# gau-nernst/llama-x

Hardware: AMD Instinct MI355X
Metric: train tokens/sec Llama-3.1-8B seq4096 at 1/2/4/8 MI355X; p50 step ms (higher is better)
Workload: dtype bf16; 1 GPU; Llama-3.1-8B text-only LoRA r=16 bf16, seq=4096, 1 sequence per GPU, causal mask, base+LM head frozen (BASELINE.json configs[1]); random-init weights at 8B dimensions; seq_len=4096, parallelism=dp1, launch=hipGraph replay (fwd+bwd+AdamW), lm_head_rows=labelled only

## Files before the change

llama-x_amd/csrc/common.h:

```cpp
#pragma once
#include <hip/hip_runtime.h>
#include <stdint.h>
#include <stdarg.h>
#include <stdio.h>

#define LLX_OK 0
#define LLX_ERR_ARG -1
#define LLX_ERR_LAUNCH -2
#define LLX_ERR_UNSUPPORTED -3

void llx_set_error(const char* fmt, ...);

#define LLX_REQUIRE(cond, ...)            \
  do {                                    \
    if (!(cond)) {                        \
      llx_set_error(__VA_ARGS__);         \
      return LLX_ERR_ARG;                 \
    }                                     \
  } while (0)

#define LLX_LAUNCH_CHECK(name)                                              \
  do {                                                                      \
    hipError_t e__ = hipGetLastError();                                     \
    if (e__ != hipSuccess) {                                                \
      llx_set_error("%s: launch failed: %s", name, hipGetErrorString(e__)); \
      return LLX_ERR_LAUNCH;                                                \
    }                                                                       \
  } while (0)

typedef uint16_t bf16_t;

typedef __attribute__((ext_vector_type(8))) __bf16 bf16x8_t;
typedef __attribute__((ext_vector_type(4))) float f32x4_t;
typedef __attribute__((ext_vector_type(16))) float f32x16_t;
typedef __attribute__((ext_vector_type(4))) int i32x4_t;
typedef __attribute__((ext_vector_type(16))) int i32x16_t;
typedef __attribute__((ext_vector_type(4))) short s16x4_t;
typedef __attribute__((ext_vector_type(4))) uint32_t u32x4_t;
typedef __attribute__((ext_vector_type(2))) uint32_t u32x2_t;

#define LLX_WAVE 64

__device__ __forceinline__ float bf2f(bf16_t v) { return __uint_as_float(((uint32_t)v) << 16); }
__device__ __forceinline__ bf16_t f2bf(float f) {
  __bf16 b = (__bf16)f;
  return __builtin_bit_cast(bf16_t, b);
}
__device__ __forceinline__ uint32_t pack_bf2(float lo, float hi) {
  return (uint32_t)f2bf(lo) | ((uint32_t)f2bf(hi) << 16);
}
__device__ __forceinline__ float bflo(uint32_t w) { return __uint_as_float(w << 16); }
__device__ __forceinline__ float bfhi(uint32_t w) { return __uint_as_float(w & 0xffff0000u); }

__device__ __forceinline__ float wave_sum(float v) {
#pragma unroll
  for (int o = 32; o > 0; o >>= 1) v += __shfl_xor(v, o, 64);
  return v;
}
__device__ __forceinline__ float wave_max(float v) {
#pragma unroll
  for (int o = 32; o > 0; o >>= 1) v = fmaxf(v, __shfl_xor(v, o, 64));
  return v;
}

__device__ __forceinline__ float block_sum(float v, float* red) {
  v = wave_sum(v);
  const int lane = threadIdx.x & 63, w = threadIdx.x >> 6, nw = (blockDim.x + 63) >> 6;
  __syncthreads();
  if (lane == 0) red[w] = v;
  __syncthreads();
  float t = 0.f;
  for (int i = 0; i < nw; ++i) t += red[i];
  return t;
}
__device__ __forceinline__ float block_max(float v, float* red) {
  v = wave_max(v);
  const int lane = threadIdx.x & 63, w = threadIdx.x >> 6, nw = (blockDim.x + 63) >> 6;
  __syncthreads();
  if (lane == 0) red[w] = v;
  __syncthreads();
  float t = red[0];
  for (int i = 1; i < nw; ++i) t = fmaxf(t, red[i]);
  return t;
}

static inline int64_t cdiv64(int64_t a, int64_t b) { return (a + b - 1) / b; }

__device__ __forceinline__ float sigmoidf_(float x) { return __builtin_amdgcn_rcpf(1.f + __expf(-x)); }
__device__ __forceinline__ u32x4_t swiglu_fwd8(const u32x4_t& gv, const u32x4_t& uv) {
  u32x4_t o;
#pragma unroll
  for (int e = 0; e < 4; ++e) {
    const float g0 = bflo(gv[e]), g1 = bfhi(gv[e]);
    const float s0 = bf2f(f2bf(g0 * sigmoidf_(g0))), s1 = bf2f(f2bf(g1 * sigmoidf_(g1)));
    o[e] = pack_bf2(s0 * bflo(uv[e]), s1 * bfhi(uv[e]));
  }
  return o;
}
__device__ __forceinline__ void swiglu_bwd8(const u32x4_t& dv, const u32x4_t& gv, const u32x4_t& uv, u32x4_t& og, u32x4_t& ou) {
#pragma unroll
  for (int e = 0; e < 4; ++e) {
    float dgs[2], dus[2];
#pragma unroll
    for (int p = 0; p < 2; ++p) {
      const float gg = p ? bfhi(gv[e]) : bflo(gv[e]);
      const float uu = p ? bfhi(uv[e]) : bflo(uv[e]);
      const float dd = p ? bfhi(dv[e]) : bflo(dv[e]);
      const float sg = sigmoidf_(gg);
      const float silu = bf2f(f2bf(gg * sg));
      dus[p] = dd * silu;
      const float ds = bf2f(f2bf(dd * uu));
      dgs[p] = ds * (sg * (1.f + gg * (1.f - sg)));
    }
    og[e] = pack_bf2(dgs[0], dgs[1]);
    ou[e] = pack_bf2(dus[0], dus[1]);
  }
}

__device__ __forceinline__ u32x4_t rope8(const u32x4_t& v, const f32x4_t& t0, const f32x4_t& t1, float sign) {
  const float cs[4] = {t0[0], t0[2], t1[0], t1[2]};
  const float sn[4] = {t0[1] * sign, t0[3] * sign, t1[1] * sign, t1[3] * sign};
  u32x4_t o;
#pragma unroll
  for (int e = 0; e < 4; ++e) {
    const float x0 = bflo(v[e]), x1 = bfhi(v[e]);
    o[e] = pack_bf2(x0 * cs[e] - x1 * sn[e], x1 * cs[e] + x0 * sn[e]);
  }
  return o;
}

__device__ __forceinline__ u32x4_t rope8(const u32x4_t& v, const float* __restrict__ tp, float sign) {
  const f32x4_t t0 = *reinterpret_cast<const f32x4_t*>(tp);
  const f32x4_t t1 = *reinterpret_cast<const f32x4_t*>(tp + 4);
  const float cs[4] = {t0[0], t0[2], t1[0], t1[2]};
  const float sn[4] = {t0[1] * sign, t0[3] * sign, t1[1] * sign, t1[3] * sign};
  u32x4_t o;
#pragma unroll
  for (int e = 0; e < 4; ++e) {
    const float x0 = bflo(v[e]), x1 = bfhi(v[e]);
    o[e] = pack_bf2(x0 * cs[e] - x1 * sn[e], x1 * cs[e] + x0 * sn[e]);
  }
  return o;
}

typedef __attribute__((ext_vector_type(8))) short llx_s16x8_t;
template <int OFF>
__device__ __forceinline__ void lds_tr_read(s16x4_t& dst, uint32_t addr) {
  asm volatile("ds_read_b64_tr_b16 %0, %1 offset:%2" : "=v"(dst) : "v"(addr), "n"(OFF));
}
__device__ __forceinline__ void lds_tr_read_rt(s16x4_t& dst, uint32_t addr, int off) {
  asm volatile("ds_read_b64_tr_b16 %0, %1 offset:%2" : "=v"(dst) : "v"(addr), "n"(off));
}
template <int N>
__device__ __forceinline__ void lds_tr_wait4(s16x4_t& a, s16x4_t& b, s16x4_t& c, s16x4_t& d) {
  asm volatile("s_waitcnt lgkmcnt(%4)" : "+v"(a), "+v"(b), "+v"(c), "+v"(d) : "n"(N));
  __builtin_amdgcn_sched_barrier(0);
}
template <int N>
__device__ __forceinline__ void lds_tr_wait8(s16x4_t (&c)[4], s16x4_t (&d)[4]) {
  asm volatile("s_waitcnt lgkmcnt(%8)" : "+v"(c[0]), "+v"(c[1]), "+v"(c[2]), "+v"(c[3]), "+v"(d[0]), "+v"(d[1]), "+v"(d[2]), "+v"(d[3]) : "n"(N));
  __builtin_amdgcn_sched_barrier(0);
}
__device__ __forceinline__ bf16x8_t frag_of(const s16x4_t& lo, const s16x4_t& hi) {
  const llx_s16x8_t v = {lo[0], lo[1], lo[2], lo[3], hi[0], hi[1], hi[2], hi[3]};
  return __builtin_bit_cast(bf16x8_t, v);
}

typedef __attribute__((address_space(3))) void llx_lds_void;
__device__ __forceinline__ __amdgpu_buffer_rsrc_t lds_dma_rsrc(const void* base, uint32_t bytes) {
  return __builtin_amdgcn_make_buffer_rsrc(const_cast<void*>(base), 0, (int)bytes, 0x00020000);
}
__device__ __forceinline__ void lds_dma16(__amdgpu_buffer_rsrc_t rsrc, llx_lds_void* dst, uint32_t lane_off, uint32_t wave_off) {
  __builtin_amdgcn_raw_ptr_buffer_load_lds(rsrc, dst, 16, (int)lane_off, (int)wave_off, 0, 0);
}
```

llama-x_amd/csrc/gemm_bf16.hip:

```cpp
#include "common.h"
#include <type_traits>
#include <mutex>

#define BM 256
#define BN 256
#define BK 64
#define STAGE_BYTES (2 * 256 * BK * 2)
#define A_TILE_BYTES (256 * BK * 2)
#define EPI_ROW_BYTES 528
#define GEMM_LDS_BYTES (256 * EPI_ROW_BYTES)

enum { EPI_NONE = 0, EPI_RESIDUAL = 1, EPI_BIAS = 2, EPI_BIAS_GELU = 3, EPI_COLSCALE = 4, EPI_ROWCOLSCALE = 5, EPI_SWIGLU_BWD = 6, EPI_SWIGLU_FWD = 7, EPI_ROPE = 8, EPI_SPLITK = 9, EPI_ROWCOLSCALE_F32 = 10 };

struct GemmArgs {
  const bf16_t* A; const bf16_t* B; bf16_t* C;
  const bf16_t* A2; const bf16_t* B2;
  const bf16_t* E;
  const bf16_t* E2;
  int64_t lda, ldb, ldc, lde, lda2, ldb2;
  int M, N, K, K2;
  int grid_m, grid_n;
  int col0, col_end;
  const bf16_t* sa; const bf16_t* sb;
  const float* rope;
  int rope_S, rope_cols;
  const int* m_valid;
  float* C32;
  int splits;
};

typedef __attribute__((address_space(3))) void lds_void;
typedef const __attribute__((address_space(1))) void gbl_void;

__device__ __forceinline__ float gelu_erf(float x) { return 0.5f * x * (1.0f + erff(x * 0.70710678118654752440f)); }

template <int EPI, bool I8, int PIPE, int BNT = 256>
__global__ __launch_bounds__(512, 2) void gemm_nt_kernel(const GemmArgs g) {
  static_assert(BNT == 256 || BNT == 128, "tile width");
  static_assert(PIPE == 1, "the four-phase main loop is the only one");
  static_assert(BNT == 256 || EPI != EPI_SWIGLU_FWD, "the SwiGLU-forward epilogue needs the full tile");
  constexpr int ESZ = I8 ? 1 : 2;
  constexpr int TK = 128 / ESZ;
  constexpr int WNG = BNT / 64;
  constexpr int WR = 256 / (8 / WNG);
  constexpr int MI = WR / 16;
  constexpr int MH = MI / 2;
  constexpr int BSI = BNT / 64;
  constexpr int EROW = BNT * 2 + 16;
  extern __shared__ __attribute__((aligned(16))) char smem[];
  const int tid = threadIdx.x;
  const int lane = tid & 63;
  const int wave = __builtin_amdgcn_readfirstlane(tid >> 6);
  const int wm = wave / WNG, wn = wave % WNG;

  int grid_m = g.grid_m;
  if (g.m_valid != nullptr) grid_m = min(grid_m, (*g.m_valid + BM - 1) / BM);
  const int nsplit = EPI == EPI_SPLITK ? g.splits : 1;
  const int nwg = grid_m * g.grid_n * nsplit;
  int bid = blockIdx.x;
  if (bid >= nwg) return;
  {
    const int q = nwg >> 3, r = nwg & 7, x = bid & 7;
    bid = (x < r ? x * (q + 1) : r * (q + 1) + (x - r) * q) + (bid >> 3);
  }
  const int split = EPI == EPI_SPLITK ? bid / (grid_m * g.grid_n) : 0;
  if constexpr (EPI == EPI_SPLITK) bid -= split * (grid_m * g.grid_n);
  const int GROUP_M = 4;
  const int width = GROUP_M * g.grid_n;
  const int group = bid / width;
  const int gsz = min(grid_m - group * GROUP_M, GROUP_M);
  const int pid_m = group * GROUP_M + ((bid % width) % gsz);
  const int pid_n = (bid % width) / gsz;
  constexpr bool SPLITN = EPI == EPI_SWIGLU_FWD;
  const int halfN = g.N >> 1;
  const int m0 = pid_m * BM, n0 = SPLITN ? pid_n * (BN / 2) : g.col0 + pid_n * BNT;
  auto col_of = [&](int nl) { return SPLITN ? (nl < BN / 2 ? n0 + nl : halfN + n0 + nl - BN / 2) : min(n0 + nl, g.col_end - 1); };

  const int srow = tid >> 3;
  const int schunk = (tid & 7) ^ ((tid >> 4) & 7);
  int arow[4], brow[4];
#pragma unroll
  for (int i = 0; i < 4; ++i) {
    arow[i] = min(m0 + i * 64 + srow, g.M - 1);
    brow[i] = SPLITN ? (i < 2 ? n0 + i * 64 + srow : halfN + n0 + (i - 2) * 64 + srow) : min(n0 + (i % BSI) * 64 + srow, g.col_end - 1);
  }
  const int nk1 = g.K / TK / nsplit;
  const int nk = nk1 + g.K2 / 64;
  const int kofs = split * nk1;

  uint32_t aoff[4], boff[4];
#pragma unroll
  for (int i = 0; i < 4; ++i) {
    aoff[i] = (uint32_t)((int64_t)arow[i] * g.lda * ESZ + schunk * 16);
    boff[i] = (uint32_t)((int64_t)brow[i] * g.ldb * ESZ + schunk * 16);
  }
  const __amdgpu_buffer_rsrc_t rsA = lds_dma_rsrc(g.A, (uint32_t)(((int64_t)(g.M - 1) * g.lda + g.K) * ESZ));
  const __amdgpu_buffer_rsrc_t rsB = lds_dma_rsrc(g.B, (uint32_t)(((int64_t)(g.N - 1) * g.ldb + g.K) * ESZ));

  const int frow = lane & 15;
  const int fsw = (lane >> 1) & 7;
  const int fq = lane >> 4;
  const int a_base = (wm * WR + frow) * 128;
  const int b_base = (wn * 64 + frow) * 128;
  const int slot0 = ((0 * 4 + fq) ^ fsw) * 16;
  const int slot1 = ((1 * 4 + fq) ^ fsw) * 16;

  using acc_t = typename std::conditional<I8, i32x4_t, f32x4_t>::type;
  acc_t acc[MI][4];
#pragma unroll
  for (int i = 0; i < MI; ++i)
#pragma unroll
    for (int j = 0; j < 4; ++j) acc[i][j] = acc_t{0, 0, 0, 0};

  auto stage_q = [&](auto steady_tag, int kt, int which) {
    constexpr bool steady = decltype(steady_tag)::value;
    if constexpr (!steady) {
      if (kt >= nk) return;
    }
    const int half = which >> 1, hi = which & 1;
    const int np = half ? BSI / 2 : 2;
    char* sT = smem + (kt & 1) * STAGE_BYTES + half * A_TILE_BYTES + hi * np * 8192;
    if (steady || kt < nk1) {
      const uint32_t koff = (uint32_t)(kt + kofs) * 128;
#pragma unroll
      for (int j = 0; j < 2; ++j) {
        if (j < np) {
          if (half) lds_dma16(rsB, (llx_lds_void*)(sT + (j * 512 + wave * 64) * 16), boff[np * hi + j], koff);
          else lds_dma16(rsA, (llx_lds_void*)(sT + (j * 512 + wave * 64) * 16), aoff[2 * hi + j], koff);
        }
      }
    } else {
      const char* base = (const char*)(half ? g.B2 : g.A2) + (int64_t)(kt - nk1) * 128;
      const int64_t l = (half ? g.ldb2 : g.lda2) * 2;
#pragma unroll
      for (int j = 0; j < 2; ++j) {
        if (j < np) {
          const char* src = base + (int64_t)(half ? brow[np * hi + j] : arow[2 * hi + j]) * l + schunk * 16;
          __builtin_amdgcn_global_load_lds((gbl_void*)src, (lds_void*)(sT + (j * 512 + wave * 64) * 16), 16, 0, 0);
        }
      }
    }
  };
  auto mfma_t = [&](auto ext_tag, const i32x4_t& b, const i32x4_t& a, acc_t& c) {
    constexpr bool ext_phase = decltype(ext_tag)::value;
    if constexpr (I8) {
      if constexpr (ext_phase) {
        f32x4_t cf = __builtin_bit_cast(f32x4_t, c);
        cf = __builtin_amdgcn_mfma_f32_16x16x32_bf16(__builtin_bit_cast(bf16x8_t, b), __builtin_bit_cast(bf16x8_t, a), cf, 0, 0, 0);
        c = __builtin_bit_cast(acc_t, cf);
      } else {
        c = __builtin_amdgcn_mfma_i32_16x16x64_i8(b, a, c, 0, 0, 0);
      }
    } else {
      c = __builtin_amdgcn_mfma_f32_16x16x32_bf16(__builtin_bit_cast(bf16x8_t, b), __builtin_bit_cast(bf16x8_t, a), c, 0, 0, 0);
    }
  };
  auto dequant_in_place = [&]() {
    if constexpr (I8) {
      float sbv[4][4], rsv[MI];
#pragma unroll
      for (int ni = 0; ni < 4; ++ni)
#pragma unroll
        for (int e = 0; e < 4; ++e) sbv[ni][e] = bf2f(g.sb[col_of(wn * 64 + ni * 16 + fq * 4 + e)]);
#pragma unroll
      for (int mi = 0; mi < MI; ++mi) rsv[mi] = bf2f(g.sa[min(m0 + wm * WR + mi * 16 + frow, g.M - 1)]);
#pragma unroll
      for (int mi = 0; mi < MI; ++mi) {
        const float rs = rsv[mi];
#pragma unroll
        for (int ni = 0; ni < 4; ++ni) {
          f32x4_t cf;
#pragma unroll
          for (int e = 0; e < 4; ++e) cf[e] = bf2f(f2bf(((float)acc[mi][ni][e] * rs) * sbv[ni][e]));
          acc[mi][ni] = __builtin_bit_cast(acc_t, cf);
        }
      }
    }
  };
  {
    const std::false_type guarded{};
    stage_q(guarded, 0, 0); stage_q(guarded, 0, 1); stage_q(guarded, 0, 2); stage_q(guarded, 0, 3);
    stage_q(guarded, 1, 2); stage_q(guarded, 1, 3); stage_q(guarded, 1, 0);
  }
  auto ktile = [&](int kt, auto ext_tag, auto steady_tag) __attribute__((always_inline)) {
    constexpr bool steady = decltype(steady_tag)::value;
    auto mfma = [&](const i32x4_t& b, const i32x4_t& a, acc_t& c) { mfma_t(ext_tag, b, a, c); };
    const char* sA = smem + (kt & 1) * STAGE_BYTES;
    const char* sB = sA + A_TILE_BYTES;
    if (steady || kt + 1 < nk) {
      if constexpr (BSI == 4) asm volatile("s_waitcnt vmcnt(6)" ::: "memory");
      else asm volatile("s_waitcnt vmcnt(4)" ::: "memory");
    } else asm volatile("s_waitcnt vmcnt(0)" ::: "memory");
    __builtin_amdgcn_s_barrier();
    asm volatile("" ::: "memory");
    stage_q(steady_tag, kt + 1, 1);
    i32x4_t bfr[2][4], af[2 * MH];
#pragma unroll
    for (int ks = 0; ks < 2; ++ks)
#pragma unroll
      for (int ni = 0; ni < 4; ++ni) bfr[ks][ni] = *reinterpret_cast<const i32x4_t*>(sB + b_base + ni * 16 * 128 + (ks ? slot1 : slot0));
#pragma unroll
    for (int ks = 0; ks < 2; ++ks)
#pragma unroll
      for (int m4 = 0; m4 < MH; ++m4) af[ks * MH + m4] = *reinterpret_cast<const i32x4_t*>(sA + a_base + m4 * 16 * 128 + (ks ? slot1 : slot0));
    __builtin_amdgcn_s_setprio(1);
#pragma unroll
    for (int ks = 0; ks < 2; ++ks)
#pragma unroll
      for (int m4 = 0; m4 < MH; ++m4)
#pragma unroll
        for (int n2 = 0; n2 < 2; ++n2) mfma(bfr[ks][n2], af[ks * MH + m4], acc[m4][n2]);
    __builtin_amdgcn_s_setprio(0);
    asm volatile("" ::: "memory");
    __builtin_amdgcn_s_barrier();
    asm volatile("" ::: "memory");
    stage_q(steady_tag, kt + 2, 2);
    __builtin_amdgcn_s_setprio(1);
#pragma unroll
    for (int ks = 0; ks < 2; ++ks)
#pragma unroll
      for (int m4 = 0; m4 < MH; ++m4)
#pragma unroll
        for (int n2 = 0; n2 < 2; ++n2) mfma(bfr[ks][2 + n2], af[ks * MH + m4], acc[m4][2 + n2]);
    __builtin_amdgcn_s_setprio(0);
    stage_q(steady_tag, kt + 2, 3);
#pragma unroll
    for (int ks = 0; ks < 2; ++ks)
#pragma unroll
      for (int m4 = 0; m4 < MH; ++m4) af[ks * MH + m4] = *reinterpret_cast<const i32x4_t*>(sA + a_base + (MH + m4) * 16 * 128 + (ks ? slot1 : slot0));
    __builtin_amdgcn_s_setprio(1);
#pragma unroll
    for (int ks = 0; ks < 2; ++ks)
#pragma unroll
      for (int m4 = 0; m4 < MH; ++m4)
#pragma unroll
        for (int n2 = 0; n2 < 2; ++n2) mfma(bfr[ks][2 + n2], af[ks * MH + m4], acc[MH + m4][2 + n2]);
    __builtin_amdgcn_s_setprio(0);
    asm volatile("" ::: "memory");
    __builtin_amdgcn_s_barrier();
    asm volatile("" ::: "memory");
    stage_q(steady_tag, kt + 2, 0);
    __builtin_amdgcn_s_setprio(1);
#pragma unroll
    for (int ks = 0; ks < 2; ++ks)
#pragma unroll
      for (int m4 = 0; m4 < MH; ++m4)
#pragma unroll
        for (int n2 = 0; n2 < 2; ++n2) mfma(bfr[ks][n2], af[ks * MH + m4], acc[MH + m4][n2]);
    __builtin_amdgcn_s_setprio(0);
  };
  const int nk_main = I8 ? nk1 : nk;
  int kt = 0;
#pragma unroll 1
  for (; kt + 2 < nk1; ++kt) ktile(kt, std::false_type{}, std::true_type{});
#pragma unroll 1
  for (; kt < nk_main; ++kt) ktile(kt, std::false_type{}, std::false_type{});
  if constexpr (I8) {
    if (nk > nk1) {
      dequant_in_place();
      for (kt = nk1; kt < nk; ++kt) ktile(kt, std::true_type{}, std::false_type{});
    }
  }
  __syncthreads();

  if constexpr (EPI == EPI_SPLITK) {
    float* P = g.C32 + (int64_t)split * g.M * g.N;
#pragma unroll
    for (int mi = 0; mi < MI; ++mi) {
      const int gm = m0 + wm * WR + mi * 16 + frow;
#pragma unroll
      for (int ni = 0; ni < 4; ++ni) {
        const int gn = n0 + wn * 64 + ni * 16 + fq * 4;
        if (gm < g.M && gn < g.col_end) *reinterpret_cast<f32x4_t*>(P + (int64_t)gm * g.N + gn) = acc[mi][ni];
      }
    }
    return;
  }
  if constexpr (EPI == EPI_ROWCOLSCALE_F32) {
    static_assert(I8, "int8 kernel only");
    float* Cf = reinterpret_cast<float*>(g.C);
    const float* saf = reinterpret_cast<const float*>(g.sa);
    const float* sbf = reinterpret_cast<const float*>(g.sb);
#pragma unroll
    for (int mi = 0; mi < MI; ++mi) {
      const int gm = m0 + wm * WR + mi * 16 + frow;
      const float rs = saf[min(gm, g.M - 1)];
#pragma unroll
      for (int ni = 0; ni < 4; ++ni) {
        const int gn = n0 + wn * 64 + ni * 16 + fq * 4;
        if (gm < g.M && gn < g.col_end) {
          const f32x4_t cs = *reinterpret_cast<const f32x4_t*>(sbf + gn);
          f32x4_t c;
#pragma unroll
          for (int e = 0; e < 4; ++e) c[e] = ((float)acc[mi][ni][e] * rs) * cs[e];
          *reinterpret_cast<f32x4_t*>(Cf + (int64_t)gm * g.ldc + gn) = c;
        }
      }
    }
    return;
  }
  constexpr int NIT = BNT / 16;
  constexpr int EB0 = (EPI == EPI_SWIGLU_BWD || EPI == EPI_ROPE) ? 4 : 8;
  constexpr int EB = EB0 < NIT / 2 ? EB0 : NIT / 2;
  constexpr bool AUX = EPI == EPI_RESIDUAL || EPI == EPI_BIAS || EPI == EPI_BIAS_GELU || EPI == EPI_SWIGLU_BWD || EPI == EPI_ROPE || EPI == EPI_COLSCALE;
  auto load_aux = [&](int it0, u32x4_t (&aux0)[EB], u32x4_t (&aux1)[EB]) {
    if constexpr (AUX) {
#pragma unroll
      for (int j = 0; j < EB; ++j) {
        const int q = (it0 + j) * 512 + tid;
        const int row = q / (BNT / 8), cc = q % (BNT / 8);
        const int gmc = min(m0 + row, g.M - 1), gnc = min(n0 + cc * 8, g.col_end - 8);
        if constexpr (EPI == EPI_RESIDUAL) {
          aux0[j] = *reinterpret_cast<const u32x4_t*>(g.E + (int64_t)gmc * g.lde + gnc);
        } else if constexpr (EPI == EPI_SWIGLU_BWD) {
          aux0[j] = *reinterpret_cast<const u32x4_t*>(g.E + (int64_t)gmc * g.lde + gnc);
          aux1[j] = *reinterpret_cast<const u32x4_t*>(g.E + (int64_t)gmc * g.lde + g.N + gnc);
        } else if constexpr (EPI == EPI_ROPE) {
          const float* tp = g.rope + ((int64_t)(gmc % g.rope_S) * 64 + ((gnc & 127) >> 1)) * 2;
          aux0[j] = *reinterpret_cast<const u32x4_t*>(tp);
          aux1[j] = *reinterpret_cast<const u32x4_t*>(tp + 4);
        } else {
          aux0[j] = *reinterpret_cast<const u32x4_t*>(g.E + gnc);
        }
      }
    }
  };
  u32x4_t auxA0[EB], auxA1[EB], auxB0[EB], auxB1[EB];
  if constexpr (!SPLITN) load_aux(0, auxA0, auxA1);
  float sbv[4][4], rsv[MI];
  if constexpr (I8) {
    if (g.K2 <= 0) {
#pragma unroll
      for (int ni = 0; ni < 4; ++ni)
#pragma unroll
        for (int e = 0; e < 4; ++e) sbv[ni][e] = bf2f(g.sb[col_of(wn * 64 + ni * 16 + fq * 4 + e)]);
#pragma unroll
      for (int mi = 0; mi < MI; ++mi) rsv[mi] = bf2f(g.sa[min(m0 + wm * WR + mi * 16 + frow, g.M - 1)]);
    }
  }
#pragma unroll
  for (int mi = 0; mi < MI; ++mi) {
    const int m = wm * WR + mi * 16 + frow;
    float rs = 1.f;
    if constexpr (I8) rs = rsv[mi];
#pragma unroll
    for (int ni = 0; ni < 4; ++ni) {
      const int n = wn * 64 + ni * 16 + fq * 4;
      float c[4];
      if constexpr (I8) {
        if (g.K2 > 0) {
          const f32x4_t cf = __builtin_bit_cast(f32x4_t, acc[mi][ni]);
#pragma unroll
          for (int e = 0; e < 4; ++e) c[e] = cf[e];
        } else {
#pragma unroll
          for (int e = 0; e < 4; ++e) c[e] = ((float)acc[mi][ni][e] * rs) * sbv[ni][e];
        }
      } else {
#pragma unroll
        for (int e = 0; e < 4; ++e) c[e] = acc[mi][ni][e];
      }
      u32x2_t pk;
      pk[0] = pack_bf2(c[0], c[1]);
      pk[1] = pack_bf2(c[2], c[3]);
      *reinterpret_cast<u32x2_t*>(smem + m * EROW + n * 2) = pk;
    }
  }
  __syncthreads();
  if constexpr (SPLITN) {
    bf16_t* H = const_cast<bf16_t*>(g.E);
#pragma unroll 4
    for (int it = 0; it < 8; ++it) {
      const int q = it * 512 + tid;
      const int row = q >> 4, cc = q & 15;
      const int gm = m0 + row, gn = n0 + cc * 8;
      if (gm < g.M) {
        const u32x4_t gv = *reinterpret_cast<const u32x4_t*>(smem + row * EPI_ROW_BYTES + cc * 16);
        const u32x4_t uv = *reinterpret_cast<const u32x4_t*>(smem + row * EPI_ROW_BYTES + (cc + 16) * 16);
        *reinterpret_cast<u32x4_t*>(g.C + (int64_t)gm * g.ldc + gn) = gv;
        *reinterpret_cast<u32x4_t*>(g.C + (int64_t)gm * g.ldc + halfN + gn) = uv;
        *reinterpret_cast<u32x4_t*>(H + (int64_t)gm * g.lde + gn) = swiglu_fwd8(gv, uv);
      }
    }
    return;
  }
  auto combine = [&](int it0, const u32x4_t (&aux0)[EB], const u32x4_t (&aux1)[EB]) {
#pragma unroll
    for (int j = 0; j < EB; ++j) {
      const int q = (it0 + j) * 512 + tid;
      const int row = q / (BNT / 8), cc = q % (BNT / 8);
      const int gm = m0 + row, gn = n0 + cc * 8;
      if (gm < g.M && gn < g.col_end) {
        u32x4_t v = *reinterpret_cast<const u32x4_t*>(smem + row * EROW + cc * 16);
        if constexpr (EPI == EPI_RESIDUAL) {
          const u32x4_t r = aux0[j];
#pragma unroll
          for (int e = 0; e < 4; ++e) v[e] = pack_bf2(bflo(v[e]) + bflo(r[e]), bfhi(v[e]) + bfhi(r[e]));
        } else if constexpr (EPI == EPI_BIAS || EPI == EPI_BIAS_GELU) {
          const u32x4_t bb = aux0[j];
#pragma unroll
          for (int e = 0; e < 4; ++e) {
            float lo = bflo(v[e]) + bflo(bb[e]), hi = bfhi(v[e]) + bfhi(bb[e]);
            if constexpr (EPI == EPI_BIAS_GELU) {
              lo = gelu_erf(bf2f(f2bf(lo)));
              hi = gelu_erf(bf2f(f2bf(hi)));
            }
            v[e] = pack_bf2(lo, hi);
          }
        } else if constexpr (EPI == EPI_SWIGLU_BWD) {
          u32x4_t og, ou;
          swiglu_bwd8(v, aux0[j], aux1[j], og, ou);
          *reinterpret_cast<u32x4_t*>(g.C + (int64_t)gm * g.ldc + g.N + gn) = ou;
          v = og;
        } else if constexpr (EPI == EPI_ROPE) {
          if (gn < g.rope_cols) v = rope8(v, __builtin_bit_cast(f32x4_t, aux0[j]), __builtin_bit_cast(f32x4_t, aux1[j]), 1.f);
        } else if constexpr (EPI == EPI_COLSCALE) {
          const u32x4_t sc = aux0[j];
#pragma unroll
          for (int e = 0; e < 4; ++e) v[e] = pack_bf2(bflo(v[e]) * bflo(sc[e]), bfhi(v[e]) * bfhi(sc[e]));
        }
        *reinterpret_cast<u32x4_t*>(g.C + (int64_t)gm * g.ldc + gn) = v;
      }
    }
  };
  static_assert((NIT / EB) % 2 == 0, "the batches alternate between two register sets");
#pragma unroll 1
  for (int it0 = 0; it0 < NIT; it0 += 2 * EB) {
    load_aux(it0 + EB, auxB0, auxB1);
    combine(it0, auxA0, auxA1);
    if (it0 + 2 * EB < NIT) load_aux(it0 + 2 * EB, auxA0, auxA1);
    combine(it0 + EB, auxB0, auxB1);
  }
}

template <int EPI, bool I8, int BNT = 256>
static int launch_gemm_p(const GemmArgs& a, hipStream_t stream) {
  auto kern = gemm_nt_kernel<EPI, I8, 1, BNT>;
  static std::once_flag attr_once;
  static hipError_t attr_err = hipSuccess;
  std::call_once(attr_once, [&] { attr_err = hipFuncSetAttribute((const void*)kern, hipFuncAttributeMaxDynamicSharedMemorySize, GEMM_LDS_BYTES); });
  if (attr_err != hipSuccess) {
    llx_set_error("llx_gemm_nt_bf16: cannot raise dynamic LDS limit: %s", hipGetErrorString(attr_err));
    return LLX_ERR_LAUNCH;
  }
  hipLaunchKernelGGL(kern, dim3(a.grid_m * a.grid_n * (EPI == EPI_SPLITK ? a.splits : 1)), dim3(512), GEMM_LDS_BYTES, stream, a);
  LLX_LAUNCH_CHECK("llx_gemm_nt_bf16");
  return LLX_OK;
}

template <int EPI, bool I8 = false>
static int launch_gemm(const GemmArgs& a, hipStream_t stream) {
  if constexpr (EPI != EPI_SWIGLU_FWD) {
    const int tiles = a.grid_m * a.grid_n, tail = tiles % 256;
    if (a.col0 == 0 && a.col_end == a.N && a.N % 256 == 0 && tiles > 256 && tail > 0 && tail <= 128 && tail % a.grid_m == 0) {
      const int tail_cols = tail / a.grid_m * 256;
      GemmArgs full = a, half = a;
      full.col_end = a.N - tail_cols;
      full.grid_n = a.grid_n - tail / a.grid_m;
      half.col0 = a.N - tail_cols;
      half.grid_n = tail_cols / 128;
      const int rc = launch_gemm_p<EPI, I8, 256>(full, stream);
      if (rc != LLX_OK) return rc;
      return launch_gemm_p<EPI, I8, 128>(half, stream);
    }
  }
  return launch_gemm_p<EPI, I8>(a, stream);
}

static GemmArgs make_args(const void* A, int64_t lda, const void* B, int64_t ldb, void* C, int64_t ldc, int64_t M, int64_t N, int64_t K) {
  GemmArgs a = {};
  a.A = (const bf16_t*)A; a.B = (const bf16_t*)B; a.C = (bf16_t*)C;
  a.lda = lda; a.ldb = ldb; a.ldc = ldc;
  a.M = (int)M; a.N = (int)N; a.K = (int)K;
  a.grid_m = (int)cdiv64(M, BM); a.grid_n = (int)cdiv64(N, BN);
  a.col_end = (int)N;
  a.splits = 1;
  return a;
}

static int check_extent(const char* who, int64_t M, int64_t N, int64_t K, int64_t lda, int64_t ldb, int esz) {
  LLX_REQUIRE(M < (1 << 30) && N < (1 << 30) && K < (1 << 30), "%s: dimension too large", who);
  LLX_REQUIRE(M * lda * esz < (int64_t)4294967296 && N * ldb * esz < (int64_t)4294967296, "%s: operand larger than 4 GiB (32-bit tile offsets)", who);
  return LLX_OK;
}

static int gemm_nt_bf16_impl(const void* A, int64_t lda, const void* B, int64_t ldb, void* C, int64_t ldc, int64_t M,
                             int64_t N, int64_t K, const void* A2, int64_t lda2, const void* B2, int64_t ldb2, int64_t K2,
                             int epilogue, const void* E, int64_t lde, const float* rope, int64_t rope_S, int64_t rope_cols,
                             hipStream_t stream, const int32_t* m_valid = nullptr) {
  LLX_REQUIRE(A && B && C, "llx_gemm_nt_bf16: null pointer");
  LLX_REQUIRE(M > 0 && N > 0 && K > 0, "llx_gemm_nt_bf16: empty problem M=%lld N=%lld K=%lld", (long long)M, (long long)N, (long long)K);
  LLX_REQUIRE(K % BK == 0 && K2 % BK == 0, "llx_gemm_nt_bf16: K=%lld and K2=%lld must be multiples of 64", (long long)K, (long long)K2);
  LLX_REQUIRE(N % 8 == 0, "llx_gemm_nt_bf16: N=%lld must be a multiple of 8", (long long)N);
  LLX_REQUIRE(lda % 8 == 0 && ldb % 8 == 0 && ldc % 8 == 0, "llx_gemm_nt_bf16: row strides must be multiples of 8 elements");
  LLX_REQUIRE(((uintptr_t)A | (uintptr_t)B | (uintptr_t)C) % 16 == 0, "llx_gemm_nt_bf16: pointers must be 16-byte aligned");
  LLX_REQUIRE(K2 == 0 || (A2 && B2 && lda2 % 8 == 0 && ldb2 % 8 == 0 && ((uintptr_t)A2 | (uintptr_t)B2) % 16 == 0),
              "llx_gemm_nt_bf16: bad K-extension operands");
  LLX_REQUIRE(epilogue == EPI_NONE || epilogue == EPI_ROPE || (E && (uintptr_t)E % 16 == 0), "llx_gemm_nt_bf16: epilogue operand missing/unaligned");
  LLX_REQUIRE(epilogue != EPI_ROPE || (rope && (uintptr_t)rope % 16 == 0 && rope_S > 0 && rope_cols >= 0 && rope_cols <= N && rope_cols % 128 == 0),
              "llx_gemm_nt_bf16_rope: need an aligned fp32 table, rope_S > 0 and rope_cols a multiple of 128 within N");
  LLX_REQUIRE((epilogue != EPI_RESIDUAL && epilogue != EPI_SWIGLU_BWD) || lde % 8 == 0, "llx_gemm_nt_bf16: residual / gate|up stride must be a multiple of 8");
  LLX_REQUIRE(epilogue != EPI_SWIGLU_BWD || (lde >= 2 * N && ldc >= 2 * N), "llx_gemm_nt_bf16: the SwiGLU-backward epilogue reads E[M,2N] (gate|up) and writes C[M,2N] (dg|du)");
  if (const int rc = check_extent("llx_gemm_nt_bf16", M, N, K, lda, ldb, 2); rc != LLX_OK) return rc;
  GemmArgs a = make_args(A, lda, B, ldb, C, ldc, M, N, K);
  a.A2 = (const bf16_t*)A2; a.B2 = (const bf16_t*)B2; a.lda2 = lda2; a.ldb2 = ldb2; a.K2 = (int)K2;
  a.E = (const bf16_t*)E; a.lde = lde;
  a.rope = rope; a.rope_S = (int)rope_S; a.rope_cols = (int)rope_cols;
  a.m_valid = m_valid;
  switch (epilogue) {
    case EPI_NONE: return launch_gemm<EPI_NONE>(a, stream);
    case EPI_RESIDUAL: return launch_gemm<EPI_RESIDUAL>(a, stream);
    case EPI_BIAS: return launch_gemm<EPI_BIAS>(a, stream);
    case EPI_BIAS_GELU: return launch_gemm<EPI_BIAS_GELU>(a, stream);
    case EPI_COLSCALE: return launch_gemm<EPI_COLSCALE>(a, stream);
    case EPI_SWIGLU_BWD: return launch_gemm<EPI_SWIGLU_BWD>(a, stream);
    case EPI_ROPE: return launch_gemm<EPI_ROPE>(a, stream);
    case EPI_SWIGLU_FWD:
      LLX_REQUIRE(N % 256 == 0 && lde % 8 == 0, "llx_gemm_nt_bf16: the SwiGLU-forward epilogue needs N = 2I with I a multiple of 128");
      a.grid_n = (int)(N / 256);
      return launch_gemm<EPI_SWIGLU_FWD>(a, stream);
    default: llx_set_error("llx_gemm_nt_bf16: unknown epilogue %d", epilogue); return LLX_ERR_UNSUPPORTED;
  }
}

extern "C" int llx_gemm_nt_bf16(const void* A, int64_t lda, const void* B, int64_t ldb, void* C, int64_t ldc, int64_t M,
                                int64_t N, int64_t K, const void* A2, int64_t lda2, const void* B2, int64_t ldb2, int64_t K2,
                                int epilogue, const void* E, int64_t lde, hipStream_t stream) {
  LLX_REQUIRE(epilogue != EPI_ROPE, "llx_gemm_nt_bf16: the RoPE epilogue is llx_gemm_nt_bf16_rope");
  return gemm_nt_bf16_impl(A, lda, B, ldb, C, ldc, M, N, K, A2, lda2, B2, ldb2, K2, epilogue, E, lde, nullptr, 0, 0, stream);
}

extern "C" int llx_gemm_nt_bf16_rows(const void* A, int64_t lda, const void* B, int64_t ldb, void* C, int64_t ldc, int64_t M,
                                     int64_t N, int64_t K, const void* A2, int64_t lda2, const void* B2, int64_t ldb2, int64_t K2,
                                     int epilogue, const void* E, int64_t lde, const int32_t* m_valid, hipStream_t stream) {
  LLX_REQUIRE(epilogue != EPI_ROPE, "llx_gemm_nt_bf16_rows: the RoPE epilogue is llx_gemm_nt_bf16_rope");
  LLX_REQUIRE(m_valid && (uintptr_t)m_valid % 4 == 0, "llx_gemm_nt_bf16_rows: m_valid must be a device int32 pointer");
  return gemm_nt_bf16_impl(A, lda, B, ldb, C, ldc, M, N, K, A2, lda2, B2, ldb2, K2, epilogue, E, lde, nullptr, 0, 0, stream, m_valid);
}

extern "C" int llx_gemm_nt_bf16_splitk(const void* A, int64_t lda, const void* B, int64_t ldb, float* partial, int64_t M, int64_t N,
                                       int64_t K, int splits, const int32_t* m_valid, hipStream_t stream) {
  LLX_REQUIRE(A && B && partial, "llx_gemm_nt_bf16_splitk: null pointer");
  LLX_REQUIRE(M > 0 && N > 0 && K > 0 && splits >= 1 && splits <= 16, "llx_gemm_nt_bf16_splitk: bad sizes");
  LLX_REQUIRE(K % ((int64_t)BK * splits) == 0, "llx_gemm_nt_bf16_splitk: K=%lld must be a multiple of 64 * splits (%d)", (long long)K, splits);
  LLX_REQUIRE(N % 8 == 0 && lda % 8 == 0 && ldb % 8 == 0, "llx_gemm_nt_bf16_splitk: N and the row strides must be multiples of 8");
  LLX_REQUIRE(((uintptr_t)A | (uintptr_t)B | (uintptr_t)partial) % 16 == 0, "llx_gemm_nt_bf16_splitk: pointers must be 16-byte aligned");
  if (const int rc = check_extent("llx_gemm_nt_bf16_splitk", M, N, K, lda, ldb, 2); rc != LLX_OK) return rc;
  LLX_REQUIRE(m_valid == nullptr || (uintptr_t)m_valid % 4 == 0, "llx_gemm_nt_bf16_splitk: m_valid must be a device int32 pointer");
  GemmArgs a = make_args(A, lda, B, ldb, nullptr, N, M, N, K);
  a.m_valid = m_valid;
  a.C32 = partial; a.splits = splits;
  return launch_gemm_p<EPI_SPLITK, false>(a, stream);
}

__global__ __launch_bounds__(256) void splitk_combine_kernel(const float* __restrict__ partial, int splits, int64_t MN, const int32_t* __restrict__ inv,
                                                             const float* __restrict__ scale, bf16_t* __restrict__ out, int64_t ldo, int N) {
  const int i = blockIdx.x, j = inv ? inv[i] : i;
  const float sc = scale ? scale[0] : 1.f;
  for (int c = threadIdx.x; c < (N >> 2); c += 256) {
    u32x2_t o = {0u, 0u};
    if (j >= 0) {
      f32x4_t v = *reinterpret_cast<const f32x4_t*>(partial + (int64_t)j * N + c * 4);
      for (int s2 = 1; s2 < splits; ++s2) {
        const f32x4_t w = *reinterpret_cast<const f32x4_t*>(partial + s2 * MN + (int64_t)j * N + c * 4);
#pragma unroll
        for (int e = 0; e < 4; ++e) v[e] += w[e];
      }
      if (scale) {
#pragma unroll
        for (int e = 0; e < 4; ++e) v[e] = bf2f(f2bf(v[e])) * sc;
      }
      o[0] = pack_bf2(v[0], v[1]);
      o[1] = pack_bf2(v[2], v[3]);
    }
    *reinterpret_cast<u32x2_t*>(out + (int64_t)i * ldo + c * 4) = o;
  }
}

extern "C" int llx_splitk_combine(const float* partial, int splits, int64_t M, int64_t N, const int32_t* inv, const float* scale, void* out,
                                  int64_t ld_out, hipStream_t stream) {
  LLX_REQUIRE(partial && out, "llx_splitk_combine: null pointer");
  LLX_REQUIRE(M > 0 && N > 0 && N % 4 == 0 && ld_out % 4 == 0 && splits >= 1 && splits <= 16, "llx_splitk_combine: bad sizes");
  LLX_REQUIRE(((uintptr_t)partial) % 16 == 0 && ((uintptr_t)out) % 8 == 0, "llx_splitk_combine: unaligned pointer");
  hipLaunchKernelGGL(splitk_combine_kernel, dim3((unsigned)M), dim3(256), 0, stream, partial, splits, M * N, inv, scale, (bf16_t*)out, ld_out, (int)N);
  LLX_LAUNCH_CHECK("llx_splitk_combine");
  return LLX_OK;
}

extern "C" int llx_gemm_nt_bf16_rope(const void* A, int64_t lda, const void* B, int64_t ldb, void* C, int64_t ldc, int64_t M, int64_t N,
                                     int64_t K, const void* A2, int64_t lda2, const void* B2, int64_t ldb2, int64_t K2,
                                     const float* rope_table, int64_t rope_S, int64_t rope_cols, hipStream_t stream) {
  return gemm_nt_bf16_impl(A, lda, B, ldb, C, ldc, M, N, K, A2, lda2, B2, ldb2, K2, EPI_ROPE, nullptr, 0, rope_table, rope_S, rope_cols, stream);
}

extern "C" int llx_int8_mm_dequant(const void* A, int64_t lda, const void* B, int64_t ldb, void* C, int64_t ldc, int64_t M, int64_t N,
                                   int64_t K, const void* a_scale, const void* b_scale, hipStream_t stream) {
  LLX_REQUIRE(A && B && C && a_scale && b_scale, "llx_int8_mm_dequant: null pointer");
  LLX_REQUIRE(M > 0 && N > 0 && K > 0, "llx_int8_mm_dequant: empty problem");
  LLX_REQUIRE(K % 128 == 0, "llx_int8_mm_dequant: K=%lld must be a multiple of 128", (long long)K);
  LLX_REQUIRE(N % 8 == 0 && ldc % 8 == 0, "llx_int8_mm_dequant: N and ldc must be multiples of 8");
  LLX_REQUIRE(lda % 16 == 0 && ldb % 16 == 0, "llx_int8_mm_dequant: int8 row strides must be multiples of 16");
  LLX_REQUIRE(((uintptr_t)A | (uintptr_t)B | (uintptr_t)C) % 16 == 0, "llx_int8_mm_dequant: pointers must be 16-byte aligned");
  if (const int rc = check_extent("llx_int8_mm_dequant", M, N, K, lda, ldb, 1); rc != LLX_OK) return rc;
  GemmArgs a = make_args(A, lda, B, ldb, C, ldc, M, N, K);
  a.sa = (const bf16_t*)a_scale; a.sb = (const bf16_t*)b_scale;
  return launch_gemm<EPI_ROWCOLSCALE, true>(a, stream);
}

extern "C" int llx_int8_mm_dequant_f32(const void* A, int64_t lda, const void* B, int64_t ldb, float* C, int64_t ldc, int64_t M, int64_t N,
                                       int64_t K, const float* a_scale, const float* b_scale, hipStream_t stream) {
  LLX_REQUIRE(A && B && C && a_scale && b_scale, "llx_int8_mm_dequant_f32: null pointer");
  LLX_REQUIRE(M > 0 && N > 0 && K > 0, "llx_int8_mm_dequant_f32: empty problem");
  LLX_REQUIRE(K % 128 == 0, "llx_int8_mm_dequant_f32: K=%lld must be a multiple of 128", (long long)K);
  LLX_REQUIRE(N % 8 == 0 && ldc % 4 == 0, "llx_int8_mm_dequant_f32: N must be a multiple of 8 and ldc of 4");
  LLX_REQUIRE(lda % 16 == 0 && ldb % 16 == 0, "llx_int8_mm_dequant_f32: int8 row strides must be multiples of 16");
  LLX_REQUIRE(((uintptr_t)A | (uintptr_t)B | (uintptr_t)C | (uintptr_t)b_scale) % 16 == 0 && (uintptr_t)a_scale % 4 == 0, "llx_int8_mm_dequant_f32: unaligned pointer");
  if (const int rc = check_extent("llx_int8_mm_dequant_f32", M, N, K, lda, ldb, 1); rc != LLX_OK) return rc;
  GemmArgs a = make_args(A, lda, B, ldb, C, ldc, M, N, K);
  a.sa = (const bf16_t*)a_scale; a.sb = (const bf16_t*)b_scale;
  return launch_gemm<EPI_ROWCOLSCALE_F32, true>(a, stream);
}

extern "C" int llx_int8_mm_dequant_ext(const void* A, int64_t lda, const void* B, int64_t ldb, void* C, int64_t ldc, int64_t M, int64_t N,
                                       int64_t K, const void* a_scale, const void* b_scale, const void* A2, int64_t lda2, const void* B2,
                                       int64_t ldb2, int64_t K2, int epilogue, const void* E, int64_t lde, const float* rope_table,
                                       int64_t rope_S, int64_t rope_cols, hipStream_t stream) {
  LLX_REQUIRE(A && B && C && a_scale && b_scale, "llx_int8_mm_dequant_ext: null pointer");
  LLX_REQUIRE(M > 0 && N > 0 && K > 0 && K2 >= 0, "llx_int8_mm_dequant_ext: empty problem");
  LLX_REQUIRE(K % 128 == 0 && K2 % 64 == 0, "llx_int8_mm_dequant_ext: K=%lld must be a multiple of 128 and K2=%lld of 64", (long long)K, (long long)K2);
  LLX_REQUIRE(N % 8 == 0 && ldc % 8 == 0, "llx_int8_mm_dequant_ext: N and ldc must be multiples of 8");
  LLX_REQUIRE(lda % 16 == 0 && ldb % 16 == 0, "llx_int8_mm_dequant_ext: int8 row strides must be multiples of 16");
  LLX_REQUIRE(((uintptr_t)A | (uintptr_t)B | (uintptr_t)C) % 16 == 0, "llx_int8_mm_dequant_ext: pointers must be 16-byte aligned");
  LLX_REQUIRE(K2 == 0 || (A2 && B2 && lda2 % 8 == 0 && ldb2 % 8 == 0 && ((uintptr_t)A2 | (uintptr_t)B2) % 16 == 0), "llx_int8_mm_dequant_ext: bad K-extension operands");
  LLX_REQUIRE(epilogue == EPI_NONE || epilogue == EPI_RESIDUAL || epilogue == EPI_SWIGLU_FWD || epilogue == EPI_ROPE, "llx_int8_mm_dequant_ext: epilogue %d unsupported", epilogue);
  LLX_REQUIRE(epilogue == EPI_NONE || epilogue == EPI_ROPE || (E && (uintptr_t)E % 16 == 0 && lde % 8 == 0), "llx_int8_mm_dequant_ext: epilogue operand missing/unaligned");
  LLX_REQUIRE(epilogue != EPI_ROPE || (rope_table && (uintptr_t)rope_table % 16 == 0 && rope_S > 0 && rope_cols >= 0 && rope_cols <= N && rope_cols % 128 == 0),
              "llx_int8_mm_dequant_ext: bad RoPE arguments");
  LLX_REQUIRE(epilogue != EPI_SWIGLU_FWD || N % 256 == 0, "llx_int8_mm_dequant_ext: the SwiGLU epilogue needs N = 2I with I a multiple of 128");
  if (const int rc = check_extent("llx_int8_mm_dequant_ext", M, N, K, lda, ldb, 1); rc != LLX_OK) return rc;
  GemmArgs a = make_args(A, lda, B, ldb, C, ldc, M, N, K);
  a.sa = (const bf16_t*)a_scale; a.sb = (const bf16_t*)b_scale;
  a.A2 = (const bf16_t*)A2; a.B2 = (const bf16_t*)B2; a.lda2 = lda2; a.ldb2 = ldb2; a.K2 = (int)K2;
  a.E = (const bf16_t*)E; a.lde = lde;
  a.rope = rope_table; a.rope_S = (int)rope_S; a.rope_cols = (int)rope_cols;
  switch (epilogue) {
    case EPI_RESIDUAL: return launch_gemm<EPI_RESIDUAL, true>(a, stream);
    case EPI_ROPE: return launch_gemm<EPI_ROPE, true>(a, stream);
    case EPI_SWIGLU_FWD: a.grid_n = (int)(N / 256); return launch_gemm<EPI_SWIGLU_FWD, true>(a, stream);
    default: return launch_gemm<EPI_ROWCOLSCALE, true>(a, stream);
  }
}
```

Before: 32120 tokens/s.

## Hand-schedule LDS fragment reads with partial lgkmcnt waits in GEMM k-loop

Replaces compiler-generated LDS loads in the bf16 GEMM main loop with inline-asm ds_read_b128 at precomputed LDS addresses, then uses graded s_waitcnt lgkmcnt waits so MFMAs on the first k-slice start before the other fragment loads finish. For the non-int8 path it also issues the upper-half A fragment reads earlier, right after the barrier, into a separate register set. The aim is to hide LDS latency behind MFMA work. In exchange it adds register pressure and relies on hand-counted wait values and sched_barrier pinning, which must match the number of reads issued.

Measured after the change: 32630 tokens/s (median of 6 runs). +1.6%, better.

```diff
diff --git a/llama-x_amd/csrc/common.h b/llama-x_amd/csrc/common.h
--- a/llama-x_amd/csrc/common.h
+++ b/llama-x_amd/csrc/common.h
@@ -161,6 +161,27 @@
   asm volatile("s_waitcnt lgkmcnt(%8)" : "+v"(c[0]), "+v"(c[1]), "+v"(c[2]), "+v"(c[3]), "+v"(d[0]), "+v"(d[1]), "+v"(d[2]), "+v"(d[3]) : "n"(N));
   __builtin_amdgcn_sched_barrier(0);
 }
+__device__ __forceinline__ void lds_read16_rt(i32x4_t& dst, uint32_t addr, int off) {
+  asm volatile("ds_read_b128 %0, %1 offset:%2" : "=v"(dst) : "v"(addr), "n"(off));
+}
+template <typename T>
+__device__ __forceinline__ void lds_pin1(T& x) { asm volatile("" : "+v"(x)); }
+template <typename T, int N>
+__device__ __forceinline__ void lds_pin1(T (&x)[N]) {
+#pragma unroll
+  for (int i = 0; i < N; ++i) asm volatile("" : "+v"(x[i]));
+}
+template <typename... T>
+__device__ __forceinline__ void lds_pin(T&... x) {
+  (lds_pin1(x), ...);
+  __builtin_amdgcn_sched_barrier(0);
+}
+template <int N, typename... T>
+__device__ __forceinline__ void lds_wait(T&... x) {
+  asm volatile("s_waitcnt lgkmcnt(%0)" : : "n"(N));
+  (lds_pin1(x), ...);
+  __builtin_amdgcn_sched_barrier(0);
+}
 __device__ __forceinline__ bf16x8_t frag_of(const s16x4_t& lo, const s16x4_t& hi) {
   const llx_s16x8_t v = {lo[0], lo[1], lo[2], lo[3], hi[0], hi[1], hi[2], hi[3]};
   return __builtin_bit_cast(bf16x8_t, v);
diff --git a/llama-x_amd/csrc/gemm_bf16.hip b/llama-x_amd/csrc/gemm_bf16.hip
--- a/llama-x_amd/csrc/gemm_bf16.hip
+++ b/llama-x_amd/csrc/gemm_bf16.hip
@@ -104,6 +104,10 @@
   const int b_base = (wn * 64 + frow) * 128;
   const int slot0 = ((0 * 4 + fq) ^ fsw) * 16;
   const int slot1 = ((1 * 4 + fq) ^ fsw) * 16;
+  const uint32_t sbase = (uint32_t)(uintptr_t)(__attribute__((address_space(3))) char*)smem;
+  const uint32_t fa0 = sbase + a_base + slot0, fa1 = sbase + a_base + slot1;
+  const uint32_t fb0 = sbase + A_TILE_BYTES + b_base + slot0, fb1 = sbase + A_TILE_BYTES + b_base + slot1;
+  constexpr bool EARLY_AHI = !I8;
 
   using acc_t = typename std::conditional<I8, i32x4_t, f32x4_t>::type;
   acc_t acc[MI][4];
@@ -185,8 +189,14 @@
   auto ktile = [&](int kt, auto ext_tag, auto steady_tag) __attribute__((always_inline)) {
     constexpr bool steady = decltype(steady_tag)::value;
     auto mfma = [&](const i32x4_t& b, const i32x4_t& a, acc_t& c) { mfma_t(ext_tag, b, a, c); };
-    const char* sA = smem + (kt & 1) * STAGE_BYTES;
-    const char* sB = sA + A_TILE_BYTES;
+    auto pin_acc = [&](int m_lo, int n_lo) {
+#pragma unroll
+      for (int m4 = 0; m4 < MH; ++m4)
+#pragma unroll
+        for (int n2 = 0; n2 < 2; ++n2) lds_pin1(acc[m_lo + m4][n_lo + n2]);
+    };
+    const uint32_t so = (uint32_t)(kt & 1) * STAGE_BYTES;
+    const uint32_t pa0 = so + fa0, pa1 = so + fa1, pb0 = so + fb0, pb1 = so + fb1;
     if (steady || kt + 1 < nk) {
       if constexpr (BSI == 4) asm volatile("s_waitcnt vmcnt(6)" ::: "memory");
       else asm volatile("s_waitcnt vmcnt(4)" ::: "memory");
@@ -194,47 +204,71 @@
     __builtin_amdgcn_s_barrier();
     asm volatile("" ::: "memory");
     stage_q(steady_tag, kt + 1, 1);
-    i32x4_t bfr[2][4], af[2 * MH];
+    i32x4_t bfr[2][4], af[2][MH], ah0[MH];
+#pragma unroll
+    for (int ks = 0; ks < 2; ++ks) {
+#pragma unroll
+      for (int n2 = 0; n2 < 2; ++n2) lds_read16_rt(bfr[ks][n2], ks ? pb1 : pb0, n2 * 16 * 128);
+#pragma unroll
+      for (int m4 = 0; m4 < MH; ++m4) lds_read16_rt(af[ks][m4], ks ? pa1 : pa0, m4 * 16 * 128);
+    }
 #pragma unroll
     for (int ks = 0; ks < 2; ++ks)
 #pragma unroll
-      for (int ni = 0; ni < 4; ++ni) bfr[ks][ni] = *reinterpret_cast<const i32x4_t*>(sB + b_base + ni * 16 * 128 + (ks ? slot1 : slot0));
-#pragma unroll
-    for (int ks = 0; ks < 2; ++ks)
-#pragma unroll
-      for (int m4 = 0; m4 < MH; ++m4) af[ks * MH + m4] = *reinterpret_cast<const i32x4_t*>(sA + a_base + m4 * 16 * 128 + (ks ? slot1 : slot0));
+      for (int n2 = 0; n2 < 2; ++n2) lds_read16_rt(bfr[ks][2 + n2], ks ? pb1 : pb0, (2 + n2) * 16 * 128);
     __builtin_amdgcn_s_setprio(1);
-#pragma unroll
-    for (int ks = 0; ks < 2; ++ks)
-#pragma unroll
-      for (int m4 = 0; m4 < MH; ++m4)
-#pragma unroll
-        for (int n2 = 0; n2 < 2; ++n2) mfma(bfr[ks][n2], af[ks * MH + m4], acc[m4][n2]);
+    lds_wait<MH + 6>(bfr[0][0], bfr[0][1], af[0]);
+#pragma unroll
+    for (int m4 = 0; m4 < MH; ++m4)
+#pragma unroll
+      for (int n2 = 0; n2 < 2; ++n2) mfma(bfr[0][n2], af[0][m4], acc[m4][n2]);
+    pin_acc(0, 0);
+    lds_wait<4>(bfr[1][0], bfr[1][1], af[1]);
+#pragma unroll
+    for (int m4 = 0; m4 < MH; ++m4)
+#pragma unroll
+      for (int n2 = 0; n2 < 2; ++n2) mfma(bfr[1][n2], af[1][m4], acc[m4][n2]);
     __builtin_amdgcn_s_setprio(0);
+    lds_wait<0>(bfr[0][2], bfr[0][3], bfr[1][2], bfr[1][3]);
     asm volatile("" ::: "memory");
     __builtin_amdgcn_s_barrier();
     asm volatile("" ::: "memory");
     stage_q(steady_tag, kt + 2, 2);
+    if constexpr (EARLY_AHI) {
+#pragma unroll
+      for (int m4 = 0; m4 < MH; ++m4) lds_read16_rt(ah0[m4], pa0, (MH + m4) * 16 * 128);
+      __builtin_amdgcn_sched_barrier(0);
+    }
     __builtin_amdgcn_s_setprio(1);
 #pragma unroll
     for (int ks = 0; ks < 2; ++ks)
 #pragma unroll
       for (int m4 = 0; m4 < MH; ++m4)
 #pragma unroll
-        for (int n2 = 0; n2 < 2; ++n2) mfma(bfr[ks][2 + n2], af[ks * MH + m4], acc[m4][2 + n2]);
+        for (int n2 = 0; n2 < 2; ++n2) mfma(bfr[ks][2 + n2], af[ks][m4], acc[m4][2 + n2]);
     __builtin_amdgcn_s_setprio(0);
     stage_q(steady_tag, kt + 2, 3);
-#pragma unroll
-    for (int ks = 0; ks < 2; ++ks)
-#pragma unroll
-      for (int m4 = 0; m4 < MH; ++m4) af[ks * MH + m4] = *reinterpret_cast<const i32x4_t*>(sA + a_base + (MH + m4) * 16 * 128 + (ks ? slot1 : slot0));
+    pin_acc(0, 2);
+    lds_pin(af[0], af[1]);
+    i32x4_t (&ah)[MH] = EARLY_AHI ? ah0 : af[0];
+    if constexpr (!EARLY_AHI) {
+#pragma unroll
+      for (int m4 = 0; m4 < MH; ++m4) lds_read16_rt(af[0][m4], pa0, (MH + m4) * 16 * 128);
+    }
+#pragma unroll
+    for (int m4 = 0; m4 < MH; ++m4) lds_read16_rt(af[1][m4], pa1, (MH + m4) * 16 * 128);
     __builtin_amdgcn_s_setprio(1);
-#pragma unroll
-    for (int ks = 0; ks < 2; ++ks)
-#pragma unroll
-      for (int m4 = 0; m4 < MH; ++m4)
-#pragma unroll
-        for (int n2 = 0; n2 < 2; ++n2) mfma(bfr[ks][2 + n2], af[ks * MH + m4], acc[MH + m4][2 + n2]);
+    lds_wait<MH>(ah);
+#pragma unroll
+    for (int m4 = 0; m4 < MH; ++m4)
+#pragma unroll
+      for (int n2 = 0; n2 < 2; ++n2) mfma(bfr[0][2 + n2], ah[m4], acc[MH + m4][2 + n2]);
+    pin_acc(MH, 2);
+    lds_wait<0>(af[1]);
+#pragma unroll
+    for (int m4 = 0; m4 < MH; ++m4)
+#pragma unroll
+      for (int n2 = 0; n2 < 2; ++n2) mfma(bfr[1][2 + n2], af[1][m4], acc[MH + m4][2 + n2]);
     __builtin_amdgcn_s_setprio(0);
     asm volatile("" ::: "memory");
     __builtin_amdgcn_s_barrier();
@@ -246,7 +280,7 @@
 #pragma unroll
       for (int m4 = 0; m4 < MH; ++m4)
 #pragma unroll
-        for (int n2 = 0; n2 < 2; ++n2) mfma(bfr[ks][n2], af[ks * MH + m4], acc[MH + m4][n2]);
+        for (int n2 = 0; n2 < 2; ++n2) mfma(bfr[ks][n2], ks ? af[1][m4] : ah[m4], acc[MH + m4][n2]);
     __builtin_amdgcn_s_setprio(0);
   };
   const int nk_main = I8 ? nk1 : nk;
```
